# Wp-Zhang/HandyRec

Measured on NVIDIA B200. Metric: DeepFM train samples/s, higher is better.
Workload: dtype f32

## Files before the change

### handyrec_b200/_lib.py

```python
from __future__ import annotations

import ctypes
import os
import re
from typing import Dict, List, Tuple

HERE = os.path.dirname(os.path.abspath(__file__))
HEADER = os.path.join(HERE, "..", "include", "hrb200.h")
LIB_PATH = os.path.join(HERE, "libhrb200.so")

HRB_OK, HRB_BAD_ARG, HRB_UNSUPPORTED, HRB_CUDA_ERROR, HRB_WORKSPACE = 0, 1, 2, 3, 4
POOL = {"none": 0, None: 0, "mean": 1, "sum": 2, "max": 3}
ACT = {None: 0, "linear": 0, "relu": 1, "sigmoid": 2, "tanh": 3, "dice": 4}
OPT_SGD, OPT_ADAM_LAZY, OPT_ADAGRAD, OPT_FTRL = 0, 1, 2, 3
GEMM_AUTO, GEMM_FP32, GEMM_3XTF32 = 0, 1, 2
BWD_AUTO, BWD_UNITS, BWD_SORT = 0, 1, 2


class HrbError(RuntimeError):
    def __init__(self, status: int, fn: str, detail: str):
        self.status = status
        super().__init__(f"{fn} failed with status {status}: {detail}")


class TableDesc(ctypes.Structure):
    _fields_ = [
        ("weight", ctypes.c_void_p),
        ("adam_m", ctypes.c_void_p),
        ("adam_v", ctypes.c_void_p),
        ("rows", ctypes.c_int64),
        ("dim", ctypes.c_int32),
        ("pad_", ctypes.c_int32),
    ]


class FieldDesc(ctypes.Structure):
    _fields_ = [
        ("table", ctypes.c_int32),
        ("seq_len", ctypes.c_int32),
        ("pool", ctypes.c_int32),
        ("ids_col", ctypes.c_int32),
        ("out_col", ctypes.c_int32),
        ("pad_", ctypes.c_int32),
    ]


class OptParams(ctypes.Structure):
    _fields_ = [
        ("opt", ctypes.c_int32),
        ("lr", ctypes.c_float),
        ("beta1", ctypes.c_float),
        ("beta2", ctypes.c_float),
        ("eps", ctypes.c_float),
        ("l2_scale", ctypes.c_float),
        ("bias_corr1", ctypes.c_float),
        ("bias_corr2", ctypes.c_float),
        ("l1", ctypes.c_float),
        ("l2", ctypes.c_float),
        ("lr_power", ctypes.c_float),
        ("l2_shrinkage", ctypes.c_float),
    ]


_SCALARS = {
    "int": ctypes.c_int,
# ... 56 lines not shown
```

### handyrec_b200/csrc/common.cuh

```cuda
#pragma once
#include <cuda_runtime.h>
#include <stdint.h>
#include <stdio.h>
#include <string.h>

#include "../../include/hrb200.h"

#define HRB_API extern "C" __attribute__((visibility("default")))

namespace hrb {

char* err_buf();
int fail(int status, const char* fmt, ...);

#define HRB_REQUIRE(cond, ...)                              \
  do {                                                      \
    if (!(cond)) return ::hrb::fail(HRB_BAD_ARG, __VA_ARGS__); \
  } while (0)

#define HRB_CUDA(call)                                                                          \
  do {                                                                                          \
    cudaError_t e_ = (call);                                                                    \
    if (e_ != cudaSuccess)                                                                      \
      return ::hrb::fail(HRB_CUDA_ERROR, "%s:%d %s -> %s", __FILE__, __LINE__, #call,           \
                         cudaGetErrorString(e_));                                               \
  } while (0)

#define HRB_LAUNCH_CHECK()             \
  do {                                 \
    ::hrb::count_launches(1);          \
    HRB_CUDA(cudaGetLastError());      \
  } while (0)

inline bool aligned16(const void* p) { return (reinterpret_cast<uintptr_t>(p) & 15u) == 0; }

void count_launches(int n);
int sm_count();

__device__ __forceinline__ float4 ldg_nc_na(const float4* p) {
  float4 r;
  asm volatile("ld.global.nc.L1::no_allocate.v4.f32 {%0,%1,%2,%3}, [%4];"
               : "=f"(r.x), "=f"(r.y), "=f"(r.z), "=f"(r.w)
               : "l"(p));
  return r;
}
__device__ __forceinline__ void stg_na(float4* p, const float4& v) {
  asm volatile("st.global.L1::no_allocate.v4.f32 [%0], {%1,%2,%3,%4};" ::"l"(p), "f"(v.x), "f"(v.y),
               "f"(v.z), "f"(v.w)
               : "memory");
}

__host__ __device__ __forceinline__ uint32_t hash_u32(uint32_t x) {
  x ^= x >> 16;
  x *= 0x7FEB352Du;
  x ^= x >> 15;
  x *= 0x846CA68Bu;
  x ^= x >> 16;
  return x;
}

__device__ __forceinline__ float warp_sum(float v) {
#pragma unroll
  for (int o = 16; o > 0; o >>= 1) v += __shfl_xor_sync(0xffffffffu, v, o);
  return v;
}

__device__ __forceinline__ bool last_block(unsigned int* counter) {
  __shared__ bool last;
  __syncthreads();
  __threadfence();
  if (threadIdx.x == 0) last = atomicAdd(counter, 1u) == gridDim.x - 1;
  __syncthreads();
  if (last) __threadfence();
  return last;
}

__device__ __forceinline__ float ftrl_pow(float a, float lr_power) { return lr_power == -0.5f ? __fsqrt_rn(a) : powf(a, -lr_power); }
__device__ __forceinline__ float ftrl_elem(float w, float& acc, float& lin, float g, float lr, float l1, float l2, float lr_power,
// ... 32 lines not shown
```

### handyrec_b200/csrc/embedding_bwd.cu

```cuda
#include <cub/block/block_radix_sort.cuh>
#include <cub/block/block_scan.cuh>

#include <stdlib.h>

#include <algorithm>
#include <new>
#include <vector>

#include "plan.cuh"

namespace hrb {

constexpr int UB_THREADS = 256;
constexpr int UB_IPT = 16;
constexpr int UB_CAP = UB_THREADS * UB_IPT;
constexpr int UB_EXPECT_MAX = 3686;
constexpr int UB_MAX_COLS = 256;
constexpr int UB_MAX_BINS = 256;
constexpr int UB_BINS = 64;
constexpr int UB_STACK = 256;
constexpr int UB_WARPS = UB_THREADS / 32;
constexpr int UB_HELPERS = 4;
constexpr int UB_TILE = 4096;
constexpr int SPLIT_ROUNDS = UB_TILE / UB_WARPS / 32;
// ... 335 lines not shown
    }
    stage_n += __popc(bal);
  };
  auto flush = [&]() {
    __syncwarp();
    for (int j0 = 0; j0 < stage_n; j0 += E * UB_APPLY) {
      int64_t rr[UB_APPLY];
      float4 vv[UB_APPLY];
      bool ok[UB_APPLY];
#pragma unroll
      for (int u = 0; u < UB_APPLY; ++u) {
        const int j = j0 + u * E + e;
        ok[u] = j < stage_n;
        rr[u] = ok[u] ? row0 + s.stage_row[w][j] : 0;
        vv[u] = ok[u] ? s.stage_acc[w][j * G + q] : make_float4(0.f, 0.f, 0.f, 0.f);
      }
      if (!HRB_UDBG(2)) apply_table_rows<MODE, UB_APPLY>(T, a.opt, a.lr_t, rr, ok, q, vv);
    }
    stage_n = 0;
    __syncwarp();
  };
  for (int k0 = seg_lo; k0 < seg_hi; k0 += E * U) {
    uint32_t r[U];
    float4 g[U];
#pragma unroll
    for (int u = 0; u < U; ++u) {
      const int i = k0 + u * E + e;
      r[u] = UB_INVALID;
      g[u] = make_float4(0.f, 0.f, 0.f, 0.f);
      if (i < seg_hi) {
        r[u] = s.row[i];
        if (!HRB_UDBG(4)) g[u] = unit_load_grad<G>(a, s.cols, s.pos[i], q);
      }
    }
#pragma unroll
    for (int u = 0; u < U; ++u) {
      const int nvalid = min(E, seg_hi - (k0 + u * E));
      if (nvalid <= 0) continue;
      const int e_end = nvalid - 1;
      float4 acc = g[u];
      const uint32_t row = r[u];
#pragma unroll
      for (int off = 1; off < E; off <<= 1) {
        const uint32_t orow = __shfl_up_sync(0xffffffffu, row, off * G);
        const float ox = __shfl_up_sync(0xffffffffu, acc.x, off * G), oy = __shfl_up_sync(0xffffffffu, acc.y, off * G);
        const float oz = __shfl_up_sync(0xffffffffu, acc.z, off * G), ow = __shfl_up_sync(0xffffffffu, acc.w, off * G);
        if (e >= off && orow == row) {
          acc.x = ox + acc.x; acc.y = oy + acc.y; acc.z = oz + acc.z; acc.w = ow + acc.w;
        }
      }
      const uint32_t rnext = __shfl_down_sync(0xffffffffu, row, G);
      const uint32_t first_row = __shfl_sync(0xffffffffu, row, q);
      if (carry_row == first_row) {
        if (row == first_row) {
          acc.x = carry.x + acc.x; acc.y = carry.y + acc.y; acc.z = carry.z + acc.z; acc.w = carry.w + acc.w;
        }
      }
      close(carry_row != first_row && carry_row != UB_NONE && e == 0, carry_row, carry);
      close(e < e_end && rnext != row, row, acc);
      carry_row = __shfl_sync(0xffffffffu, row, e_end * G + q);
      carry.x = __shfl_sync(0xffffffffu, acc.x, e_end * G + q);
      carry.y = __shfl_sync(0xffffffffu, acc.y, e_end * G + q);
      carry.z = __shfl_sync(0xffffffffu, acc.z, e_end * G + q);
      carry.w = __shfl_sync(0xffffffffu, acc.w, e_end * G + q);
    }
    flush();
// ... 532 lines not shown
```

### handyrec_b200/csrc/lookup.cu

```cuda
#include <cub/device/device_radix_sort.cuh>
#include <algorithm>
#include <new>
#include <stdlib.h>
#include <string.h>
#include <vector>

#include "common.cuh"

#include "plan.cuh"

namespace hrb {

constexpr uint32_t kNotMine = 0xFFFFFFFFu;

__global__ void __launch_bounds__(256) embedding_fwd_kernel(const float* __restrict__ table, int64_t vocab,
                                                            int32_t chunks ,
                                                            const int32_t* __restrict__ ids, int64_t n_ids,
                                                            float* __restrict__ out, uint8_t* __restrict__ mask,
                                                            int32_t* __restrict__ oob) {
  const int64_t total = n_ids * chunks;
  const int64_t stride = (int64_t)gridDim.x * blockDim.x;
  constexpr int U = 4;
  for (int64_t base = blockIdx.x * (int64_t)blockDim.x + threadIdx.x; base < total; base += stride * U) {
    int32_t id[U];
// ... 899 lines not shown
              "hrb_seq_pool_fwd: Pooling method should be `mean`, `max`, or `sum`");
  if (batch == 0) return HRB_OK;
  seq_pool_fwd_kernel<<<grid_for(batch * dim, 256), 256, 0, (cudaStream_t)stream>>>(x, mask, batch, seq_len, dim,
                                                                                    method, out);
  HRB_LAUNCH_CHECK();
  return HRB_OK;
}

HRB_API int hrb_seq_pool_bwd(const float* x, const uint8_t* mask, const float* dout, int64_t batch, int32_t seq_len,
                             int32_t dim, int32_t method, float* dx, void* stream) {
  HRB_REQUIRE(x && mask && dout && dx && batch >= 0 && seq_len > 0 && dim > 0, "hrb_seq_pool_bwd: null/negative argument");
  HRB_REQUIRE(method == HRB_POOL_MEAN || method == HRB_POOL_SUM || method == HRB_POOL_MAX,
              "hrb_seq_pool_bwd: Pooling method should be `mean`, `max`, or `sum`");
  if (batch == 0) return HRB_OK;
  seq_pool_bwd_kernel<<<grid_for(batch * dim, 256), 256, 0, (cudaStream_t)stream>>>(x, mask, dout, batch, seq_len,
                                                                                    dim, method, dx);
  HRB_LAUNCH_CHECK();
  return HRB_OK;
}

HRB_API int hrb_plan_create(const hrb_table_desc* tables_host, int32_t n_tables, const hrb_field_desc* fields_host,
                            int32_t n_fields, hrb_plan** plan_out) {
  HRB_REQUIRE(tables_host && fields_host && plan_out && n_tables > 0 && n_fields > 0, "hrb_plan_create: null/empty argument");
  hrb_plan* p = new (std::nothrow) hrb_plan();
  HRB_REQUIRE(p != nullptr, "hrb_plan_create: out of host memory");
  p->n_tables = n_tables;
  p->n_fields = n_fields;
  p->tables.assign(tables_host, tables_host + n_tables);
  p->fields.assign(fields_host, fields_host + n_fields);
  uint64_t base = 0;
  p->tdev_host.resize(n_tables);
  for (int t = 0; t < n_tables; ++t) {
    const hrb_table_desc& td = p->tables[t];
    if (!td.weight || td.rows <= 0 || td.dim <= 0 || td.dim % 4 != 0 || !aligned16(td.weight) ||
        (td.adam_m && !aligned16(td.adam_m)) || (td.adam_v && !aligned16(td.adam_v))) {
      delete p;
      return fail(td.dim % 4 ? HRB_UNSUPPORTED : HRB_BAD_ARG,
                  "hrb_plan_create: table %d needs a 16-byte aligned weight, rows>0 and dim%%4==0 (dim=%d)", t, td.dim);
    }
    p->tdev_host[t] = TableDev{td.weight, td.adam_m, td.adam_v, td.rows, (uint32_t)base, td.dim, nullptr};
    base += (uint64_t)td.rows;
    if (td.dim > p->max_dim) p->max_dim = td.dim;
  }
  if (base >= 0xFFFFFFFFull) {
    delete p;
    return fail(HRB_UNSUPPORTED, "hrb_plan_create: %llu total rows do not fit 32-bit sort keys", (unsigned long long)base);
  }
  p->total_rows = base;
  p->key_bits = bits_for(base);
  p->fdev_host.resize(n_fields);
  std::vector<int32_t> chunk_field, chunk_q, pos_field;
  const int32_t dim0 = p->tables[p->fields[0].table < n_tables && p->fields[0].table >= 0 ? p->fields[0].table : 0].dim;
  for (int f = 0; f < n_fields; ++f) {
    const hrb_field_desc& fd = p->fields[f];
    if (fd.table < 0 || fd.table >= n_tables || fd.seq_len <= 0 || fd.ids_col < 0 || fd.out_col < 0 ||
        fd.out_col % 4 != 0 || fd.pool < HRB_POOL_NONE || fd.pool > HRB_POOL_MAX ||
        (fd.pool == HRB_POOL_NONE && fd.seq_len != 1)) {
      delete p;
      return fail(HRB_BAD_ARG, "hrb_plan_create: field %d is malformed (table/seq_len/cols/pool)", f);
    }
    const TableDev& td = p->tdev_host[fd.table];
    p->fdev_host[f] = FieldDev{td.w, td.rows, td.key_base, td.dim, fd.seq_len, fd.pool, fd.ids_col, fd.out_col,
                               p->pos_cols, fd.table};
    for (int l = 0; l < fd.seq_len; ++l) pos_field.push_back(f);
    p->pos_cols += fd.seq_len;
    for (int q = 0; q < td.dim / 4; ++q) {
      chunk_field.push_back(f);
      chunk_q.push_back(q);
    }
    if (td.dim != dim0) p->uniform_dim = false;
    if (fd.out_col != p->fields[0].out_col + f * dim0) p->contiguous_out = false;
    if (fd.seq_len != 1 || fd.pool != HRB_POOL_NONE) p->all_len1 = false;
    if (fd.pool == HRB_POOL_MAX) p->has_max = true;
// ... 842 lines not shown
```

### handyrec_b200/csrc/plan.cuh

```cuda
#pragma once
#include <cstddef>
#include <mutex>
#include <vector>

#include "common.cuh"

namespace hrb {

struct FieldDev {
  const float* table;
  int64_t rows;
  uint32_t key_base;
  int32_t dim;
  int32_t seq_len;
  int32_t pool;
  int32_t ids_col;
  int32_t out_col;
  int32_t pos_col;
  int32_t table_idx;
};

struct TableDev {
  float* w;
  float* m;
  float* v;
  int64_t rows;
  uint32_t key_base;
  int32_t dim;
  float* grad;
};

enum UpdMode : int { UPD_SGD = 0, UPD_ADAM = 1, UPD_DENSE_ADD = 2, UPD_ADAGRAD = 3, UPD_FTRL = 4 };

inline int upd_mode(int32_t opt) {
  return opt == HRB_OPT_ADAM_LAZY ? UPD_ADAM : opt == HRB_OPT_ADAGRAD ? UPD_ADAGRAD : opt == HRB_OPT_FTRL ? UPD_FTRL : UPD_SGD;
}

inline hrb_opt_params load_opt(const hrb_opt_params* p) {
  hrb_opt_params o{};
  memcpy(&o, p, offsetof(hrb_opt_params, l1));
  if (o.opt == HRB_OPT_FTRL) {
    o.l1 = p->l1;
    o.l2 = p->l2;
    o.lr_power = p->lr_power;
    o.l2_shrinkage = p->l2_shrinkage;
  }
  return o;
}

__device__ __forceinline__ void ftrl_row4(float4& w, float4& a, float4& l, const float4& g, const hrb_opt_params& o) {
  w.x = ftrl_elem(w.x, a.x, l.x, g.x, o.lr, o.l1, o.l2, o.lr_power, o.l2_shrinkage);
  w.y = ftrl_elem(w.y, a.y, l.y, g.y, o.lr, o.l1, o.l2, o.lr_power, o.l2_shrinkage);
  w.z = ftrl_elem(w.z, a.z, l.z, g.z, o.lr, o.l1, o.l2, o.lr_power, o.l2_shrinkage);
  w.w = ftrl_elem(w.w, a.w, l.w, g.w, o.lr, o.l1, o.l2, o.lr_power, o.l2_shrinkage);
}

__device__ __forceinline__ void adagrad_elem(float& w, float& acc, float g, float lr, float eps) {
  acc = fmaf(g, g, acc);
  w -= lr * g / (sqrtf(acc) + eps);
}

template <int MODE>
__device__ __forceinline__ void apply_table_row(const TableDev& t, const hrb_opt_params& opt, float lr_t, int64_t row, int q, float4 g) {
  if (q * 4 >= t.dim) return;
  const int64_t off = row * (t.dim >> 2) + q;
  if (t.grad != nullptr) {
    float4* gp = reinterpret_cast<float4*>(t.grad) + off;
    float4 o = *gp;
    o.x += g.x; o.y += g.y; o.z += g.z; o.w += g.w;
    *gp = o;
    return;
  }
  float4* wp = reinterpret_cast<float4*>(t.w) + off;
  float4 w = *wp;
  if (MODE == UPD_FTRL) {
    float4* ap = reinterpret_cast<float4*>(t.m) + off;
    float4* lp = reinterpret_cast<float4*>(t.v) + off;
    float4 a = *ap, l = *lp;
    const float l2 = opt.l2_scale;
    g.x = fmaf(l2, w.x, g.x); g.y = fmaf(l2, w.y, g.y); g.z = fmaf(l2, w.z, g.z); g.w = fmaf(l2, w.w, g.w);
    ftrl_row4(w, a, l, g, opt);
    *ap = a;
    *lp = l;
    *wp = w;
    return;
  }
  const float l2 = opt.l2_scale;
  g.x = fmaf(l2, w.x, g.x); g.y = fmaf(l2, w.y, g.y); g.z = fmaf(l2, w.z, g.z); g.w = fmaf(l2, w.w, g.w);
  if (MODE == UPD_SGD) {
    const float lr = opt.lr;
    w.x -= lr * g.x; w.y -= lr * g.y; w.z -= lr * g.z; w.w -= lr * g.w;
  } else if (MODE == UPD_ADAGRAD) {
    float4* ap = reinterpret_cast<float4*>(t.m) + off;
    float4 a = *ap;
    const float lr = opt.lr, e = opt.eps;
    adagrad_elem(w.x, a.x, g.x, lr, e); adagrad_elem(w.y, a.y, g.y, lr, e);
    adagrad_elem(w.z, a.z, g.z, lr, e); adagrad_elem(w.w, a.w, g.w, lr, e);
    *ap = a;
  } else {
    float4* mp = reinterpret_cast<float4*>(t.m) + off;
    float4* vp = reinterpret_cast<float4*>(t.v) + off;
    float4 m = *mp, v = *vp;
    const float b1 = opt.beta1, b2 = opt.beta2, e = opt.eps, lr = lr_t;
    m.x = b1 * m.x + (1.f - b1) * g.x; m.y = b1 * m.y + (1.f - b1) * g.y;
    m.z = b1 * m.z + (1.f - b1) * g.z; m.w = b1 * m.w + (1.f - b1) * g.w;
    v.x = b2 * v.x + (1.f - b2) * g.x * g.x; v.y = b2 * v.y + (1.f - b2) * g.y * g.y;
    v.z = b2 * v.z + (1.f - b2) * g.z * g.z; v.w = b2 * v.w + (1.f - b2) * g.w * g.w;
    w.x -= lr * m.x / (sqrtf(v.x) + e); w.y -= lr * m.y / (sqrtf(v.y) + e);
    w.z -= lr * m.z / (sqrtf(v.z) + e); w.w -= lr * m.w / (sqrtf(v.w) + e);
    *mp = m;
    *vp = v;
  }
  *wp = w;
}

template <int MODE, int N>
__device__ __forceinline__ void apply_table_rows(const TableDev& t, const hrb_opt_params& opt, float lr_t, const int64_t (&row)[N],
                                                 const bool (&ok_in)[N], int q, float4 (&g)[N]) {
  const bool in_dim = q * 4 < t.dim;
  bool ok[N];
  int64_t off[N];
#pragma unroll
  for (int i = 0; i < N; ++i) {
    ok[i] = ok_in[i] && in_dim;
    off[i] = row[i] * (t.dim >> 2) + q;
  }
  if (t.grad != nullptr) {
    float4 o[N];
#pragma unroll
    for (int i = 0; i < N; ++i)
      if (ok[i]) o[i] = reinterpret_cast<float4*>(t.grad)[off[i]];
#pragma unroll
    for (int i = 0; i < N; ++i)
      if (ok[i]) {
        o[i].x += g[i].x; o[i].y += g[i].y; o[i].z += g[i].z; o[i].w += g[i].w;
        reinterpret_cast<float4*>(t.grad)[off[i]] = o[i];
      }
    return;
  }
  float4 w[N], m[N], v[N];
#pragma unroll
  for (int i = 0; i < N; ++i) {
    if (ok[i]) {
      w[i] = reinterpret_cast<float4*>(t.w)[off[i]];
      if (MODE != UPD_SGD) m[i] = reinterpret_cast<float4*>(t.m)[off[i]];
      if (MODE == UPD_ADAM || MODE == UPD_FTRL) v[i] = reinterpret_cast<float4*>(t.v)[off[i]];
    }
  }
  const float l2 = opt.l2_scale;
#pragma unroll
  for (int i = 0; i < N; ++i) {
    if (!ok[i]) continue;
    float4 gi = g[i], wi = w[i];
    gi.x = fmaf(l2, wi.x, gi.x); gi.y = fmaf(l2, wi.y, gi.y); gi.z = fmaf(l2, wi.z, gi.z); gi.w = fmaf(l2, wi.w, gi.w);
    if (MODE == UPD_SGD) {
      const float lr = opt.lr;
      wi.x -= lr * gi.x; wi.y -= lr * gi.y; wi.z -= lr * gi.z; wi.w -= lr * gi.w;
    } else if (MODE == UPD_ADAGRAD) {
      float4 ai = m[i];
      const float lr = opt.lr, e = opt.eps;
      adagrad_elem(wi.x, ai.x, gi.x, lr, e); adagrad_elem(wi.y, ai.y, gi.y, lr, e);
      adagrad_elem(wi.z, ai.z, gi.z, lr, e); adagrad_elem(wi.w, ai.w, gi.w, lr, e);
      reinterpret_cast<float4*>(t.m)[off[i]] = ai;
    } else if (MODE == UPD_FTRL) {
      float4 ai = m[i], li = v[i];
      ftrl_row4(wi, ai, li, gi, opt);
      reinterpret_cast<float4*>(t.m)[off[i]] = ai;
      reinterpret_cast<float4*>(t.v)[off[i]] = li;
    } else {
      float4 mi = m[i], vi = v[i];
      const float b1 = opt.beta1, b2 = opt.beta2, e = opt.eps, lr = lr_t;
      mi.x = b1 * mi.x + (1.f - b1) * gi.x; mi.y = b1 * mi.y + (1.f - b1) * gi.y;
      mi.z = b1 * mi.z + (1.f - b1) * gi.z; mi.w = b1 * mi.w + (1.f - b1) * gi.w;
      vi.x = b2 * vi.x + (1.f - b2) * gi.x * gi.x; vi.y = b2 * vi.y + (1.f - b2) * gi.y * gi.y;
      vi.z = b2 * vi.z + (1.f - b2) * gi.z * gi.z; vi.w = b2 * vi.w + (1.f - b2) * gi.w * gi.w;
      wi.x -= lr * mi.x / (sqrtf(vi.x) + e); wi.y -= lr * mi.y / (sqrtf(vi.y) + e);
      wi.z -= lr * mi.z / (sqrtf(vi.z) + e); wi.w -= lr * mi.w / (sqrtf(vi.w) + e);
      reinterpret_cast<float4*>(t.m)[off[i]] = mi;
      reinterpret_cast<float4*>(t.v)[off[i]] = vi;
    }
    reinterpret_cast<float4*>(t.w)[off[i]] = wi;
  }
}

struct UnitDev {
  int32_t table;
  uint32_t row_lo, row_hi;
  int32_t slice, n_slices;
  int32_t partial_idx;
  int32_t list;
  int32_t pad_;
};
struct ColDev {
  int32_t pos_col;
  int32_t out_col;
  int32_t field;
  int32_t pad_;
};
struct SliceGroupDev {
  int32_t table;
  uint32_t row;
  int32_t partial_idx, n_slices;
};
struct TableSplitDev {
  int32_t first_list, n_bins, shift;
  int32_t first_tile, n_tiles;
  uint32_t ent_base;
};
struct TileDev {
  int32_t table, col_local, pos_col, chunk;
};
struct UnitSet {
// ... 61 lines not shown
```

### handyrec_b200/engine.py

```python
from __future__ import annotations

import ctypes
import math
from typing import Dict, List, Optional, Sequence, Tuple

import numpy as np
import torch

from . import _lib
from . import kernels as K
from ._lib import call


def _r4(n: int) -> int:
    return (n + 3) // 4 * 4


def launch_count() -> int:
    c = ctypes.c_int64(0)
    call("hrb_launch_count", ctypes.byref(c))
    return c.value


class DeepFMEngine:
# ... 102 lines not shown
            self._table_off[t] = off
            off += self.tables[t].numel()
        self.n_params = off
        self.tab0 = min(self._table_off.values()) if self._table_off else off
        n_touched = (off - self.tab0) // self.D if optimizer == "ftrl" else 0
        self.params = torch.zeros(off, device=self.dev, dtype=torch.float32)
        self.grads = torch.zeros(off + n_touched + self._n_pad_flags, device=self.dev, dtype=torch.float32)
        self.touched = self.grads[off : off + n_touched] if n_touched else None
        self.opt_m = torch.zeros(off, device=self.dev, dtype=torch.float32) if optimizer == "adam" else None
        self.opt_v = torch.zeros(off, device=self.dev, dtype=torch.float32) if optimizer == "adam" else None
        if optimizer in ("adagrad", "ftrl"):
            self.opt_m = torch.full((off,), self.initial_accumulator_value, device=self.dev, dtype=torch.float32)
        if optimizer == "ftrl":
            self.opt_v = torch.zeros(off, device=self.dev, dtype=torch.float32)
        self.W, self.b, self.dW, self.db = [], [], [], []
        for (wo, bo), Kp, ld in zip(offs, self.layer_K, self.layer_ld):
            self.W.append(self.params[wo : wo + Kp * ld].view(Kp, ld))
            self.b.append(self.params[bo : bo + ld])
            self.dW.append(self.grads[wo : wo + Kp * ld].view(Kp, ld))
            self.db.append(self.grads[bo : bo + ld])
        self.fm_w = self.params[self.fm_off : self.fm_off + self.D]
        self.fm_w0 = self.params[self.fm_off + self.D : self.fm_off + self.D + 1]
        self.d_fm = self.grads[self.fm_off : self.fm_off + self.D + 1]
        self._init_dense(seed)
        table_grads: List[Optional[torch.Tensor]] = [None] * len(self.tables)
        for t, o in self._table_off.items():
            n = self.tables[t].numel()
            live = self.params[o : o + n].view_as(self.tables[t])
            live.copy_(self.tables[t])
            self.tables[t] = live
            table_grads[t] = self.grads[o : o + n].view_as(live)
        self.table_grads = table_grads
        self.adam_m = self.adam_v = self.accum = self.linear = None
        if self.emb_opt == "adam_lazy":
            self.adam_m = [None if t in self._table_off else torch.zeros_like(w) for t, w in enumerate(self.tables)]
            self.adam_v = [None if t in self._table_off else torch.zeros_like(w) for t, w in enumerate(self.tables)]
        elif self.emb_opt in ("adagrad", "ftrl"):
            self.accum = [None if t in self._table_off else torch.full_like(w, self.initial_accumulator_value) for t, w in enumerate(self.tables)]
        if self.emb_opt == "ftrl":
            self.linear = [None if t in self._table_off else torch.zeros_like(w) for t, w in enumerate(self.tables)]
        self.plan = K.LookupPlan(self.tables, plan_fields, self.adam_m, self.adam_v, accum=self.accum, linear=self.linear)
        self.table_touched: List[Optional[torch.Tensor]] = [None] * len(self.tables)
        if self.touched is not None:
            for t, o in self._table_off.items():
                r0 = (o - self.tab0) // self.D
                self.table_touched[t] = self.touched[r0 : r0 + self.tables[t].shape[0]]
        if self.dense_tables:
            self.plan.set_dense_grads(table_grads)

        B = self.B
        f32 = dict(device=self.dev, dtype=torch.float32)
        self.X0 = torch.zeros(B, self.K0p, **f32)
        self.A = [torch.zeros(B, ld, **f32) for ld in self.layer_ld]
        self.dZ = [torch.zeros(B, ld, **f32) for ld in self.layer_ld]
        self.dX0 = torch.zeros(B, self.K0p, **f32)
        self.fm_out = torch.empty(B, **f32)
        self.fm_sum = torch.empty(B, self.D, **f32)
        self.prob = torch.empty(B, **f32)
        self.loss_sum = torch.zeros(1, **f32)
        self._loss_ws = K.regression_loss_workspace(B, self.dev) if task == "regression" else None
        self.use_tc = gemm_mode != _lib.GEMM_FP32 and B >= 512 and B % 4 == 0
        self.tc_layer = [self.use_tc and u >= 16 for u in self.units]
        if self.use_tc:
            self.Wt = [torch.zeros(ld, Kp, **f32) if tc else None for ld, Kp, tc in zip(self.layer_ld, self.layer_K, self.tc_layer)]
            self.dZt = [torch.zeros(ld, B, **f32) for ld in self.layer_ld]
            self.relu_mask = [torch.zeros(B, (u + 31) // 32, device=self.dev, dtype=torch.int32) if self.act == "relu" else None for u in self.units]
            self._refresh_wt()
        self.ids_dev = torch.zeros(B, self.ids_cols, device=self.dev, dtype=torch.int32)
        self.dense_dev = torch.zeros(B, max(self.n_dense, 1), **f32)
        self.label_dev = torch.zeros(B, **f32)
        self.loss_host = torch.zeros(1, dtype=torch.float32).pin_memory()
        self._ws_emb = torch.empty(self.plan.workspace_bytes(B), device=self.dev, dtype=torch.uint8)
        self.clip = None
# ... 509 lines not shown
```

### handyrec_b200/kernels.py

```python
from __future__ import annotations

import ctypes
from typing import List, Optional, Sequence, Tuple

import torch

from . import _lib
from ._lib import ACT, POOL, FieldDesc, OptParams, TableDesc, call

__all__ = [
    "init_uniform", "embedding_fwd", "embedding_bwd_dense", "seq_pool_fwd", "seq_pool_bwd", "LookupPlan",
    "fm_fwd", "fm_bwd", "dense_fwd", "dense_bwd_x", "dense_bwd_w", "act_bwd", "dice_fwd", "dice_bwd",
    "lau_fwd", "lau_pack_params", "sigmoid_bce", "regression_loss", "regression_loss_workspace", "adam_step", "sgd_step",
    "adam_step_multi", "sgd_step_multi",
    "adagrad_step", "adagrad_step_multi", "ftrl_step", "ftrl_step_multi", "metric_scratch_bytes", "metric_weighted_scratch_bytes",
    "metric_update",
    "clip_workspace", "clip_prepare_multi", "clip_scales", "clip_apply_multi",
]


_raw_stream = getattr(torch._C, "_cuda_getCurrentRawStream", None)


def _stream() -> ctypes.c_void_p:
# ... 78 lines not shown
    n = ids.numel()
    need = ctypes.c_size_t(0)
    call("hrb_embedding_bwd_dense_workspace", n, D, ctypes.byref(need))
    ws = torch.empty(need.value, device=dout.device, dtype=torch.uint8)
    dtable = torch.empty(vocab, D, device=dout.device, dtype=torch.float32)
    call("hrb_embedding_bwd_dense", _p(ids), n, _p(dout), vocab, D, _p(table), float(l2_scale), _p(dtable), _p(ws), need.value, _stream())
    return dtable


def _mask_u8(mask: torch.Tensor) -> torch.Tensor:
    if mask.dtype == torch.bool:
        mask = mask.view(torch.uint8)
    return _chk(mask, torch.uint8, "mask")


def seq_pool_fwd(x: torch.Tensor, mask: Optional[torch.Tensor], method: str) -> torch.Tensor:
    assert method in ["mean", "max", "sum"], "Pooling method should be `mean`, `max`, or `sum`"
    if mask is None:
        raise ValueError("Embedding layer should set `mask_zero` as True")
    _chk(x, torch.float32, "x")
    B, L, D = x.shape
    out = torch.empty(B, 1, D, device=x.device, dtype=torch.float32)
    call("hrb_seq_pool_fwd", _p(x), _p(_mask_u8(mask)), B, L, D, POOL[method], _p(out), _stream())
    return out


def seq_pool_bwd(x: torch.Tensor, mask: torch.Tensor, dout: torch.Tensor, method: str) -> torch.Tensor:
    _chk(x, torch.float32, "x")
    _chk(dout, torch.float32, "dout")
    B, L, D = x.shape
    dx = torch.empty_like(x)
    call("hrb_seq_pool_bwd", _p(x), _p(_mask_u8(mask)), _p(dout), B, L, D, POOL[method], _p(dx), _stream())
    return dx


class LookupPlan:

    def __init__(self, tables: Sequence[torch.Tensor], fields: Sequence[Tuple[int, int, str, int, int]],
                 adam_m: Optional[Sequence[torch.Tensor]] = None, adam_v: Optional[Sequence[torch.Tensor]] = None,
                 accum: Optional[Sequence[torch.Tensor]] = None, linear: Optional[Sequence[torch.Tensor]] = None):
        self.tables = [_chk(t, torch.float32, "table") for t in tables]
        if accum is not None:
            if adam_m is not None:
                raise ValueError("LookupPlan: pass either adam_m (Adam) or accum (Adagrad / Ftrl), not both")
            adam_m = accum
        if linear is not None:
            if adam_v is not None:
                raise ValueError("LookupPlan: pass either adam_v (Adam) or linear (Ftrl), not both")
            adam_v = linear
        self.adam_m = list(adam_m) if adam_m is not None else None
        self.adam_v = list(adam_v) if adam_v is not None else None
        self.fields = [tuple(f) for f in fields]
        self.n_fields = len(self.fields)
        self.device = self.tables[0].device
        td = (TableDesc * len(self.tables))()
        for i, t in enumerate(self.tables):
            td[i].weight = t.data_ptr()
            td[i].adam_m = self.adam_m[i].data_ptr() if self.adam_m is not None and self.adam_m[i] is not None else 0
            td[i].adam_v = self.adam_v[i].data_ptr() if self.adam_v is not None and self.adam_v[i] is not None else 0
            td[i].rows, td[i].dim = t.shape[0], t.shape[1]
        fd = (FieldDesc * self.n_fields)()
        self.ids_cols = 0
        self.out_cols = 0
        self.pos_cols = 0
        for i, (ti, L, pool, ids_col, out_col) in enumerate(self.fields):
            fd[i].table, fd[i].seq_len, fd[i].pool, fd[i].ids_col, fd[i].out_col = ti, L, POOL[pool], ids_col, out_col
            self.ids_cols = max(self.ids_cols, ids_col + L)
            self.out_cols = max(self.out_cols, out_col + self.tables[ti].shape[1])
            self.pos_cols += L
        self._h = ctypes.c_void_p(0)
        with torch.cuda.device(self.device):
            call("hrb_plan_create", td, len(self.tables), fd, self.n_fields, ctypes.byref(self._h))
        self._ws = None

    def set_dense_grads(self, grads: Sequence[Optional[torch.Tensor]]) -> None:
        assert len(grads) == len(self.tables)
        self._dense_grads = list(grads)
        arr = (ctypes.c_void_p * len(grads))(*[(g.data_ptr() if g is not None else None) for g in grads])
        call("hrb_plan_set_dense_grads", self._h, arr)

    def mark_rows(self, ids: torch.Tensor, touched: Sequence[Optional[torch.Tensor]]) -> None:
        assert len(touched) == len(self.tables)
        ids_ld = self._ids_ld(ids)
        for t in touched:
            if t is not None:
                _chk(t, torch.float32, "touched")
        arr = (ctypes.c_void_p * len(touched))(*[(t.data_ptr() if t is not None else None) for t in touched])
        call("hrb_plan_mark_rows", self._h, _p(ids), ids_ld, ids.shape[0], arr, _stream())

    def pad_flags(self, ids: torch.Tensor, flags: torch.Tensor) -> None:
        _chk(flags, torch.float32, "flags")
        call("hrb_plan_pad_flags", self._h, _p(ids), self._ids_ld(ids), ids.shape[0], _p(flags), _stream())

# ... 503 lines not shown
```

### handyrec_b200/layers/tools.py

```python
from __future__ import annotations

from typing import List

import numpy as np
import torch

from ..autograd_ops import AttPoolFn, EmbeddingFn, MatmulNTFn, RowDotFn, SampledSoftmaxFn
from ..keras_lite import KTensor, Layer, device


class ValueTable(Layer):

    def __init__(self, value_list: List, dtype: str = "int32", **kwargs):
        self._np = np.asarray(value_list)
        self._dtype = dtype
        self.value = None
        super().__init__(**kwargs)

    def call(self, *args, **kwargs):
        if self.value is None:
            from ..keras_lite import _tdtype

            self.value = torch.as_tensor(self._np).to(device(), _tdtype(self._dtype))
        return self.value
# ... 46 lines not shown

    def call(self, inputs):
        if self._sharded is not None:
            raise RuntimeError(f"{self.name}: this table is row-sharded over {self._sharded[1]} GPUs; only the fused engine "
                               "(a DeepFM-shaped model compiled under ShardedTables / distribute=True) reads it")
        ids = inputs.to(torch.int32)
        sink = None
        rows_only = self.input_dim >= self.SPARSE_UPDATE_MIN_ROWS or (self._ftrl and not self.l2)
        if self._ftrl and not self.l2 and self.output_dim % 4 != 0 and self.trainable and torch.is_grad_enabled():
            raise ValueError(f"{self.name}: the touched-rows Ftrl update needs output_dim % 4 == 0, got {self.output_dim}")
        if self.trainable and rows_only and torch.is_grad_enabled() and self.output_dim % 4 == 0:
            if not hasattr(self, "_sparse_grads"):
                self._sparse_grads = []
            sink = self._sparse_grads
        out, mask = EmbeddingFn.apply(self.embeddings, ids, self.mask_zero, sink)
        self._last_mask = mask if self.mask_zero else None
        if not torch.is_grad_enabled():
            out._hrb_src = (self.embeddings.data, ids)
        return out

    def apply_sparse(self, optimizer) -> None:
        pending = getattr(self, "_sparse_grads", None)
        if not pending:
            return
        from .. import kernels as K
        from ..keras_lite import Adagrad, Adam, Ftrl

        ids = torch.cat([i for i, _ in pending]).reshape(-1, 1).contiguous()
        rows = torch.cat([g for _, g in pending]).contiguous()
        pending.clear()
        adam, adagrad, ftrl = isinstance(optimizer, Adam), isinstance(optimizer, Adagrad), isinstance(optimizer, Ftrl)
        if getattr(self, "_plan", None) is None:
            w = self.embeddings.data
            self._m, self._v = (torch.zeros_like(w), torch.zeros_like(w)) if adam else (None, None)
            self._accum = torch.full_like(w, optimizer.initial_accumulator_value) if (adagrad or ftrl) else None
            self._linear = torch.zeros_like(w) if ftrl else None
            self._plan = K.LookupPlan([w], [(0, 1, "none", 0, 0)], [self._m] if adam else None, [self._v] if adam else None,
                                      accum=[self._accum] if (adagrad or ftrl) else None, linear=[self._linear] if ftrl else None)
        if adam:
            self._plan.backward_update(ids, rows, opt="adam", lr=optimizer.lr_t, l2_scale=2.0 * self.l2, beta1=optimizer.b1, beta2=optimizer.b2,
                                       eps=optimizer.eps, step=max(optimizer.t, 1), autotune=True)
        elif adagrad:
            self._plan.backward_update(ids, rows, opt="adagrad", lr=optimizer.lr_t, l2_scale=2.0 * self.l2, eps=optimizer.eps, autotune=True)
        elif ftrl:
            self._plan.backward_update(ids, rows, opt="ftrl", lr=optimizer.lr_t, l2_scale=2.0 * self.l2, autotune=True, **optimizer.hyper())
        else:
            self._plan.backward_update(ids, rows, opt="sgd", lr=optimizer.lr_t, l2_scale=2.0 * self.l2, autotune=True)

    def compute_mask(self, inputs, mask=None):
        if not self.mask_zero:
            return None
        return self._last_mask

    def symbolic_has_mask(self, inputs, in_masks):
        return self.mask_zero

    def compute_output_shape(self, input_shape):
        return tuple(input_shape) + (self.output_dim,)


class SqueezeMask(Layer):

    def call(self, inputs, *args, **kwargs):
        if isinstance(inputs, KTensor):
            return inputs
        out = inputs + 0
        if hasattr(inputs, "_hrb_src"):
            out._hrb_src = inputs._hrb_src
        return out
# ... 122 lines not shown
```

### include/hrb200.h

```cpp
#ifndef HRB200_H_
#define HRB200_H_

#include <stddef.h>
#include <stdint.h>

#ifdef __cplusplus
extern "C" {
#endif

#define HRB_ABI_VERSION 1

typedef enum hrb_status {
  HRB_OK = 0,
  HRB_BAD_ARG = 1,
  HRB_UNSUPPORTED = 2,
  HRB_CUDA_ERROR = 3,
  HRB_WORKSPACE = 4
} hrb_status;

typedef enum hrb_pool { HRB_POOL_NONE = 0, HRB_POOL_MEAN = 1, HRB_POOL_SUM = 2, HRB_POOL_MAX = 3 } hrb_pool;

typedef enum hrb_act {
  HRB_ACT_LINEAR = 0,
  HRB_ACT_RELU = 1,
  HRB_ACT_SIGMOID = 2,
  HRB_ACT_TANH = 3,
  HRB_ACT_DICE = 4
} hrb_act;

int hrb_abi_version(void);
const char* hrb_status_str(int status);
const char* hrb_last_error(void);
int hrb_launch_count(int64_t* count);

int hrb_init_uniform(float* table, int64_t rows, int32_t dim, uint32_t seed, float lo, float hi,
                     int64_t row_start, int64_t row_step, void* stream);

int hrb_embedding_fwd(const float* table, int64_t vocab, int32_t dim, const int32_t* ids, int64_t n_ids,
                      float* out, uint8_t* mask, int32_t* oob, void* stream);

int hrb_embedding_bwd_dense_workspace(int64_t n_ids, int32_t dim, size_t* bytes);
int hrb_embedding_bwd_dense(const int32_t* ids, int64_t n_ids, const float* dout, int64_t vocab, int32_t dim,
                            const float* table, float l2_scale, float* dtable, void* workspace,
                            size_t workspace_bytes, void* stream);

int hrb_seq_pool_fwd(const float* x, const uint8_t* mask, int64_t batch, int32_t seq_len, int32_t dim,
                     int32_t method, float* out, void* stream);
int hrb_seq_pool_bwd(const float* x, const uint8_t* mask, const float* dout, int64_t batch, int32_t seq_len,
                     int32_t dim, int32_t method, float* dx, void* stream);

typedef struct hrb_table_desc {
  float* weight;
  float* adam_m;
  float* adam_v;
  int64_t rows;
  int32_t dim;
  int32_t pad_;
} hrb_table_desc;

typedef struct hrb_field_desc {
  int32_t table;
  int32_t seq_len;
  int32_t pool;
  int32_t ids_col;
  int32_t out_col;
  int32_t pad_;
} hrb_field_desc;

typedef struct hrb_plan hrb_plan;

int hrb_plan_create(const hrb_table_desc* tables_host, int32_t n_tables, const hrb_field_desc* fields_host,
                    int32_t n_fields, hrb_plan** plan);
int hrb_plan_destroy(hrb_plan* plan);

int hrb_lookup_fwd(const hrb_plan* plan, const int32_t* ids, int64_t ids_ld, int64_t batch, float* out,
                   int64_t out_ld, float* inv_count, int32_t* oob, void* stream);

int hrb_lookup_fm_fwd(const hrb_plan* plan, const int32_t* ids, int64_t ids_ld, int64_t batch, float* out,
                      int64_t out_ld, float* inv_count, const float* fm_w, const float* fm_w0, float* fm_out,
                      float* fm_sum, int32_t* oob, void* stream);

typedef enum hrb_opt { HRB_OPT_SGD = 0, HRB_OPT_ADAM_LAZY = 1, HRB_OPT_ADAGRAD = 2, HRB_OPT_FTRL = 3 } hrb_opt;
typedef struct hrb_opt_params {
  int32_t opt;
  float lr, beta1, beta2, eps, l2_scale;
  float bias_corr1, bias_corr2;
  float l1, l2, lr_power, l2_shrinkage;
} hrb_opt_params;
int hrb_lookup_bwd_workspace(const hrb_plan* plan, int64_t ids_ld, int64_t batch, size_t* bytes);
int hrb_lookup_bwd_update(const hrb_plan* plan, const int32_t* ids, int64_t ids_ld, int64_t batch,
// ... 208 lines not shown
```

Measured before the change: 53.86 million.

## Interleave optimizer slots per row and prefetch table rows into L2

Stores the two optimizer state tensors (Adam m/v or FTRL accum/linear) interleaved in one record per row, with a slot_ld stride, so both slots of a row sit in adjacent memory. Adds an L2 prefetch of the weight and slot rows for each unique row in the sparse backward update before the gradient accumulation runs. The goal is fewer scattered DRAM sectors and hidden latency in the row-wise optimizer update. In exchange the plan ABI and alignment rules change, and the prefetches add extra instructions that may be wasted.

After: 54.88 million, median of 6. +1.9%, better.

```diff
diff --git a/handyrec_b200/_lib.py b/handyrec_b200/_lib.py
--- a/handyrec_b200/_lib.py
+++ b/handyrec_b200/_lib.py
@@ -30,7 +30,7 @@
         ("adam_v", ctypes.c_void_p),
         ("rows", ctypes.c_int64),
         ("dim", ctypes.c_int32),
-        ("pad_", ctypes.c_int32),
+        ("slot_ld", ctypes.c_int32),
     ]
 
 
diff --git a/handyrec_b200/csrc/common.cuh b/handyrec_b200/csrc/common.cuh
--- a/handyrec_b200/csrc/common.cuh
+++ b/handyrec_b200/csrc/common.cuh
@@ -44,6 +44,7 @@
                : "l"(p));
   return r;
 }
+__device__ __forceinline__ void prefetch_l2(const void* p) { asm volatile("prefetch.global.L2 [%0];" ::"l"(p)); }
 __device__ __forceinline__ void stg_na(float4* p, const float4& v) {
   asm volatile("st.global.L1::no_allocate.v4.f32 [%0], {%1,%2,%3,%4};" ::"l"(p), "f"(v.x), "f"(v.y),
                "f"(v.z), "f"(v.w)
diff --git a/handyrec_b200/csrc/embedding_bwd.cu b/handyrec_b200/csrc/embedding_bwd.cu
--- a/handyrec_b200/csrc/embedding_bwd.cu
+++ b/handyrec_b200/csrc/embedding_bwd.cu
@@ -391,6 +391,11 @@
         r[u] = s.row[i];
         if (!HRB_UDBG(4)) g[u] = unit_load_grad<G>(a, s.cols, s.pos[i], q);
       }
+    }
+#pragma unroll
+    for (int u = 0; u < U; ++u) {
+      const int i = k0 + u * E + e;
+      if (!HRB_UDBG(2) && i < seg_hi && (i == seg_lo || s.row[i - 1] != r[u])) prefetch_table_row<MODE>(T, row0 + r[u], q);
     }
 #pragma unroll
     for (int u = 0; u < U; ++u) {
diff --git a/handyrec_b200/csrc/lookup.cu b/handyrec_b200/csrc/lookup.cu
--- a/handyrec_b200/csrc/lookup.cu
+++ b/handyrec_b200/csrc/lookup.cu
@@ -955,13 +955,18 @@
   p->tdev_host.resize(n_tables);
   for (int t = 0; t < n_tables; ++t) {
     const hrb_table_desc& td = p->tables[t];
-    if (!td.weight || td.rows <= 0 || td.dim <= 0 || td.dim % 4 != 0 || !aligned16(td.weight) ||
-        (td.adam_m && !aligned16(td.adam_m)) || (td.adam_v && !aligned16(td.adam_v))) {
+    if (!td.weight || td.rows <= 0 || td.dim <= 0 || td.dim % 4 != 0 || !aligned16(td.weight)) {
       delete p;
       return fail(td.dim % 4 ? HRB_UNSUPPORTED : HRB_BAD_ARG,
                   "hrb_plan_create: table %d needs a 16-byte aligned weight, rows>0 and dim%%4==0 (dim=%d)", t, td.dim);
     }
-    p->tdev_host[t] = TableDev{td.weight, td.adam_m, td.adam_v, td.rows, (uint32_t)base, td.dim, nullptr};
+    if ((td.adam_m || td.adam_v) && (td.slot_ld < td.dim || td.slot_ld % 4 != 0 || (td.adam_m && (uintptr_t)td.adam_m % 128 != 0) ||
+                                     (td.adam_v && !aligned16(td.adam_v)))) {
+      delete p;
+      return fail(HRB_BAD_ARG, "hrb_plan_create: table %d: optimiser slots need slot_ld %% 4 == 0, slot_ld >= dim (slot_ld=%d, dim=%d), "
+                  "adam_m 128-byte and adam_v 16-byte aligned", t, td.slot_ld, td.dim);
+    }
+    p->tdev_host[t] = TableDev{td.weight, td.adam_m, td.adam_v, td.rows, (uint32_t)base, td.dim, td.slot_ld, nullptr};
     base += (uint64_t)td.rows;
     if (td.dim > p->max_dim) p->max_dim = td.dim;
   }
diff --git a/handyrec_b200/csrc/plan.cuh b/handyrec_b200/csrc/plan.cuh
--- a/handyrec_b200/csrc/plan.cuh
+++ b/handyrec_b200/csrc/plan.cuh
@@ -27,6 +27,7 @@
   int64_t rows;
   uint32_t key_base;
   int32_t dim;
+  int32_t slot_ld;
   float* grad;
 };
 
@@ -64,6 +65,7 @@
 __device__ __forceinline__ void apply_table_row(const TableDev& t, const hrb_opt_params& opt, float lr_t, int64_t row, int q, float4 g) {
   if (q * 4 >= t.dim) return;
   const int64_t off = row * (t.dim >> 2) + q;
+  const int64_t soff = row * (t.slot_ld >> 2) + q;
   if (t.grad != nullptr) {
     float4* gp = reinterpret_cast<float4*>(t.grad) + off;
     float4 o = *gp;
@@ -74,8 +76,8 @@
   float4* wp = reinterpret_cast<float4*>(t.w) + off;
   float4 w = *wp;
   if (MODE == UPD_FTRL) {
-    float4* ap = reinterpret_cast<float4*>(t.m) + off;
-    float4* lp = reinterpret_cast<float4*>(t.v) + off;
+    float4* ap = reinterpret_cast<float4*>(t.m) + soff;
+    float4* lp = reinterpret_cast<float4*>(t.v) + soff;
     float4 a = *ap, l = *lp;
     const float l2 = opt.l2_scale;
     g.x = fmaf(l2, w.x, g.x); g.y = fmaf(l2, w.y, g.y); g.z = fmaf(l2, w.z, g.z); g.w = fmaf(l2, w.w, g.w);
@@ -91,15 +93,15 @@
     const float lr = opt.lr;
     w.x -= lr * g.x; w.y -= lr * g.y; w.z -= lr * g.z; w.w -= lr * g.w;
   } else if (MODE == UPD_ADAGRAD) {
-    float4* ap = reinterpret_cast<float4*>(t.m) + off;
+    float4* ap = reinterpret_cast<float4*>(t.m) + soff;
     float4 a = *ap;
     const float lr = opt.lr, e = opt.eps;
     adagrad_elem(w.x, a.x, g.x, lr, e); adagrad_elem(w.y, a.y, g.y, lr, e);
     adagrad_elem(w.z, a.z, g.z, lr, e); adagrad_elem(w.w, a.w, g.w, lr, e);
     *ap = a;
   } else {
-    float4* mp = reinterpret_cast<float4*>(t.m) + off;
-    float4* vp = reinterpret_cast<float4*>(t.v) + off;
+    float4* mp = reinterpret_cast<float4*>(t.m) + soff;
+    float4* vp = reinterpret_cast<float4*>(t.v) + soff;
     float4 m = *mp, v = *vp;
     const float b1 = opt.beta1, b2 = opt.beta2, e = opt.eps, lr = lr_t;
     m.x = b1 * m.x + (1.f - b1) * g.x; m.y = b1 * m.y + (1.f - b1) * g.y;
@@ -114,16 +116,34 @@
   *wp = w;
 }
 
+template <int MODE>
+__device__ __forceinline__ void prefetch_table_row(const TableDev& t, int64_t row, int q) {
+  if ((q & 7) != 0 || q * 4 >= t.dim) return;
+  if (t.grad != nullptr) {
+    prefetch_l2(t.grad + row * t.dim + 4 * q);
+    return;
+  }
+  prefetch_l2(t.w + row * t.dim + 4 * q);
+  if (MODE == UPD_SGD) return;
+  const float* mp = t.m + row * t.slot_ld + 4 * q;
+  prefetch_l2(mp);
+  if (MODE == UPD_ADAM || MODE == UPD_FTRL) {
+    const float* vp = t.v + row * t.slot_ld + 4 * q;
+    if (((uintptr_t)vp >> 7) != ((uintptr_t)mp >> 7)) prefetch_l2(vp);
+  }
+}
+
 template <int MODE, int N>
 __device__ __forceinline__ void apply_table_rows(const TableDev& t, const hrb_opt_params& opt, float lr_t, const int64_t (&row)[N],
                                                  const bool (&ok_in)[N], int q, float4 (&g)[N]) {
   const bool in_dim = q * 4 < t.dim;
   bool ok[N];
-  int64_t off[N];
+  int64_t off[N], soff[N];
 #pragma unroll
   for (int i = 0; i < N; ++i) {
     ok[i] = ok_in[i] && in_dim;
     off[i] = row[i] * (t.dim >> 2) + q;
+    soff[i] = row[i] * (t.slot_ld >> 2) + q;
   }
   if (t.grad != nullptr) {
     float4 o[N];
@@ -143,8 +163,8 @@
   for (int i = 0; i < N; ++i) {
     if (ok[i]) {
       w[i] = reinterpret_cast<float4*>(t.w)[off[i]];
-      if (MODE != UPD_SGD) m[i] = reinterpret_cast<float4*>(t.m)[off[i]];
-      if (MODE == UPD_ADAM || MODE == UPD_FTRL) v[i] = reinterpret_cast<float4*>(t.v)[off[i]];
+      if (MODE != UPD_SGD) m[i] = reinterpret_cast<float4*>(t.m)[soff[i]];
+      if (MODE == UPD_ADAM || MODE == UPD_FTRL) v[i] = reinterpret_cast<float4*>(t.v)[soff[i]];
     }
   }
   const float l2 = opt.l2_scale;
@@ -161,12 +181,12 @@
       const float lr = opt.lr, e = opt.eps;
       adagrad_elem(wi.x, ai.x, gi.x, lr, e); adagrad_elem(wi.y, ai.y, gi.y, lr, e);
       adagrad_elem(wi.z, ai.z, gi.z, lr, e); adagrad_elem(wi.w, ai.w, gi.w, lr, e);
-      reinterpret_cast<float4*>(t.m)[off[i]] = ai;
+      reinterpret_cast<float4*>(t.m)[soff[i]] = ai;
     } else if (MODE == UPD_FTRL) {
       float4 ai = m[i], li = v[i];
       ftrl_row4(wi, ai, li, gi, opt);
-      reinterpret_cast<float4*>(t.m)[off[i]] = ai;
-      reinterpret_cast<float4*>(t.v)[off[i]] = li;
+      reinterpret_cast<float4*>(t.m)[soff[i]] = ai;
+      reinterpret_cast<float4*>(t.v)[soff[i]] = li;
     } else {
       float4 mi = m[i], vi = v[i];
       const float b1 = opt.beta1, b2 = opt.beta2, e = opt.eps, lr = lr_t;
@@ -176,8 +196,8 @@
       vi.z = b2 * vi.z + (1.f - b2) * gi.z * gi.z; vi.w = b2 * vi.w + (1.f - b2) * gi.w * gi.w;
       wi.x -= lr * mi.x / (sqrtf(vi.x) + e); wi.y -= lr * mi.y / (sqrtf(vi.y) + e);
       wi.z -= lr * mi.z / (sqrtf(vi.z) + e); wi.w -= lr * mi.w / (sqrtf(vi.w) + e);
-      reinterpret_cast<float4*>(t.m)[off[i]] = mi;
-      reinterpret_cast<float4*>(t.v)[off[i]] = vi;
+      reinterpret_cast<float4*>(t.m)[soff[i]] = mi;
+      reinterpret_cast<float4*>(t.v)[soff[i]] = vi;
     }
     reinterpret_cast<float4*>(t.w)[off[i]] = wi;
   }
diff --git a/handyrec_b200/engine.py b/handyrec_b200/engine.py
--- a/handyrec_b200/engine.py
+++ b/handyrec_b200/engine.py
@@ -158,13 +158,18 @@
             table_grads[t] = self.grads[o : o + n].view_as(live)
         self.table_grads = table_grads
         self.adam_m = self.adam_v = self.accum = self.linear = None
-        if self.emb_opt == "adam_lazy":
-            self.adam_m = [None if t in self._table_off else torch.zeros_like(w) for t, w in enumerate(self.tables)]
-            self.adam_v = [None if t in self._table_off else torch.zeros_like(w) for t, w in enumerate(self.tables)]
-        elif self.emb_opt in ("adagrad", "ftrl"):
-            self.accum = [None if t in self._table_off else torch.full_like(w, self.initial_accumulator_value) for t, w in enumerate(self.tables)]
-        if self.emb_opt == "ftrl":
-            self.linear = [None if t in self._table_off else torch.zeros_like(w) for t, w in enumerate(self.tables)]
+        row_upd = [t for t in range(len(self.tables)) if t not in self._table_off]
+        if self.emb_opt in ("adam_lazy", "ftrl"):
+            first = self.initial_accumulator_value if self.emb_opt == "ftrl" else 0.0
+            rec = {t: K.slot_record(self.tables[t], first) for t in row_upd}
+            s0 = [rec[t][0] if t in rec else None for t in range(len(self.tables))]
+            s1 = [rec[t][1] if t in rec else None for t in range(len(self.tables))]
+            if self.emb_opt == "ftrl":
+                self.accum, self.linear = s0, s1
+            else:
+                self.adam_m, self.adam_v = s0, s1
+        elif self.emb_opt == "adagrad":
+            self.accum = [torch.full_like(w, self.initial_accumulator_value) if t in row_upd else None for t, w in enumerate(self.tables)]
         self.plan = K.LookupPlan(self.tables, plan_fields, self.adam_m, self.adam_v, accum=self.accum, linear=self.linear)
         self.table_touched: List[Optional[torch.Tensor]] = [None] * len(self.tables)
         if self.touched is not None:
diff --git a/handyrec_b200/kernels.py b/handyrec_b200/kernels.py
--- a/handyrec_b200/kernels.py
+++ b/handyrec_b200/kernels.py
@@ -134,6 +134,16 @@
     dx = torch.empty_like(x)
     call("hrb_seq_pool_bwd", _p(x), _p(_mask_u8(mask)), _p(dout), B, L, D, POOL[method], _p(dx), _stream())
     return dx
+
+
+def slot_record(table: torch.Tensor, first: float = 0.0) -> Tuple[torch.Tensor, torch.Tensor]:
+    rows, d = table.shape
+    rec = torch.zeros(rows, 2 * d, device=table.device, dtype=torch.float32)
+    if rec.data_ptr() % 128 != 0:
+        raise RuntimeError(f"slot_record: the allocator returned a buffer that is not 128-byte aligned ({rec.data_ptr():#x})")
+    if first != 0.0:
+        rec[:, :d].fill_(first)
+    return rec[:, :d], rec[:, d:]
 
 
 class LookupPlan:
@@ -158,9 +168,18 @@
         td = (TableDesc * len(self.tables))()
         for i, t in enumerate(self.tables):
             td[i].weight = t.data_ptr()
+            td[i].rows, td[i].dim = t.shape[0], t.shape[1]
+            slots = [s[i] for s in (self.adam_m, self.adam_v) if s is not None and s[i] is not None]
+            for s in slots:
+                if s.dtype != torch.float32 or s.device != t.device or s.shape != t.shape:
+                    raise ValueError(f"LookupPlan: optimiser slot of table {i} must be fp32 {tuple(t.shape)} on {t.device}, "
+                                     f"got {s.dtype} {tuple(s.shape)} on {s.device}")
+            lds = {_row_major_2d(s, f"optimiser slot of table {i}") for s in slots}
+            if len(lds) > 1 and t.shape[0] > 1:
+                raise ValueError(f"LookupPlan: the optimiser slots of table {i} have different row strides {sorted(lds)}")
+            td[i].slot_ld = max(lds) if lds else t.shape[1]
             td[i].adam_m = self.adam_m[i].data_ptr() if self.adam_m is not None and self.adam_m[i] is not None else 0
             td[i].adam_v = self.adam_v[i].data_ptr() if self.adam_v is not None and self.adam_v[i] is not None else 0
-            td[i].rows, td[i].dim = t.shape[0], t.shape[1]
         fd = (FieldDesc * self.n_fields)()
         self.ids_cols = 0
         self.out_cols = 0
diff --git a/handyrec_b200/layers/tools.py b/handyrec_b200/layers/tools.py
--- a/handyrec_b200/layers/tools.py
+++ b/handyrec_b200/layers/tools.py
@@ -102,9 +102,12 @@
         adam, adagrad, ftrl = isinstance(optimizer, Adam), isinstance(optimizer, Adagrad), isinstance(optimizer, Ftrl)
         if getattr(self, "_plan", None) is None:
             w = self.embeddings.data
-            self._m, self._v = (torch.zeros_like(w), torch.zeros_like(w)) if adam else (None, None)
-            self._accum = torch.full_like(w, optimizer.initial_accumulator_value) if (adagrad or ftrl) else None
-            self._linear = torch.zeros_like(w) if ftrl else None
+            self._m, self._v = K.slot_record(w) if adam else (None, None)
+            self._accum, self._linear = None, None
+            if ftrl:
+                self._accum, self._linear = K.slot_record(w, optimizer.initial_accumulator_value)
+            elif adagrad:
+                self._accum = torch.full_like(w, optimizer.initial_accumulator_value)
             self._plan = K.LookupPlan([w], [(0, 1, "none", 0, 0)], [self._m] if adam else None, [self._v] if adam else None,
                                       accum=[self._accum] if (adagrad or ftrl) else None, linear=[self._linear] if ftrl else None)
         if adam:
diff --git a/include/hrb200.h b/include/hrb200.h
--- a/include/hrb200.h
+++ b/include/hrb200.h
@@ -55,7 +55,7 @@
   float* adam_v;
   int64_t rows;
   int32_t dim;
-  int32_t pad_;
+  int32_t slot_ld;
 } hrb_table_desc;
 
 typedef struct hrb_field_desc {
```
